# refresh-bio/DSRC

Measured on AMD Instinct MI355X. Metric: raw FASTQ MB/s compressed (bit-identical .dsrc) at -d3 -q2, higher is better.
Workload: dtype u8/u16/u32 integer

## Files before the change

dsrc_amd/csrc/dsrc_gpu.hip:

```cpp
#include <hip/hip_runtime.h>

#include <algorithm>
#include <atomic>
#include <cstdarg>
#include <cstdio>
#include <cstdlib>
#include <cstring>
#include <chrono>
#include <condition_variable>
#include <deque>
#include <functional>
#include <dlfcn.h>
#include <mutex>
#ifndef DSRC_REPLAY_WHATIF
#define DSRC_REPLAY_WHATIF 0
#endif
#include <string>
#include <thread>
#include <vector>

#include "../../include/dsrc_gpu.h"
#include "dsrc_types.h"
#include "k_common.h"
#ifndef RCS_WIDE
// ... 168 lines not shown
	const char* fill = hook_env("DSRC_GPU_DEBUG_FILL");
	if (h->arena.cap >= need) { h->arena.top = 0; h->arena.failed = false; if (fill) HIPCHK(hipMemsetAsync(h->arena.base, atoi(fill), h->arena.cap, h->stream)); return 0; }
	if (h->arena_fixed && need > h->arena_fixed)
		return fail(h, DSRCGPU_E_NOMEM, "batch needs %zu bytes of HBM scratch, arena is fixed at %llu", need, (unsigned long long)h->arena_fixed);
	if (h->arena.base) { HIPCHK(hipFree(h->arena.base)); h->arena.base = nullptr; h->arena.cap = 0; }
	size_t want = h->arena_fixed ? (size_t)h->arena_fixed : need + need / 64;
	hipError_t e;
	{
		static std::mutex alloc_turn[64];
		std::lock_guard<std::mutex> g(alloc_turn[h->device & 63]);
		const auto t0 = std::chrono::steady_clock::now();
		e = hipMalloc((void**)&h->arena.base, want);
		if (getenv("DSRC_GPU_DEBUG")) fprintf(stderr, "[dsrc_gpu] %p arena of %.1f GB: hipMalloc took %.0f ms\n", (void*)h, want / 1e9, std::chrono::duration<double, std::milli>(std::chrono::steady_clock::now() - t0).count());
	}
	if (e != hipSuccess) return fail(h, DSRCGPU_E_NOMEM, "hipMalloc(%zu) for the batch arena failed: %s", want, hipGetErrorString(e));
	h->arena.cap = want; h->arena.top = 0; h->arena.failed = false;
	if (fill) HIPCHK(hipMemsetAsync(h->arena.base, atoi(fill), h->arena.cap, h->stream));
	return 0;
}

u32 bitlen(u64 x) { for (u32 i = 0; i < 32; ++i) if (x < (1ull << i)) return i; return 64; }
u32 log2u(u32 x) { u32 r = 0; while (x > 1) { x >>= 1; ++r; } return r; }
u32 h_huff_ws_words(u32 n) { const u32 m = n < 2 ? 2 : n; return 10 * m; }
u32 h_huff_tree_cap(u32 n) { const u32 m = n < 2 ? 2 : n; return (16 + (2 * m + m * 10) / 8 + 8 + 3) & ~3u; }
size_t al(size_t x, size_t a) { return (x + a - 1) / a * a; }

size_t estimate_arena(const dsrcgpu_handle* h, u32 n, const u64* sizes)
{
	const bool rc = h->set.dna_order > 0 || h->set.quality_order > 0;
	size_t tot = 0, mx = 0;
	for (u32 i = 0; i < n; ++i) { tot += (size_t)sizes[i] + 4096; mx = std::max(mx, (size_t)sizes[i]); }
	const size_t sort_slice = std::min(tot * 14, slice_budget(tot) + mx * 16);
	const size_t copy = (h->set.tag_preserve_flags || h->ds.color_space || !h->rec_pending.empty()) ? tot + (1u << 20) : 0;
	return tot * (h->rc_caps_worst ? 18 : 15) / 2 + (rc ? sort_slice : 0) + (size_t)n * (1u << 20) + (16u << 20) + copy;
}
size_t estimate_decode_arena(const dsrcgpu_handle* h, u32 n, const u64* sizes, bool own_text);

struct BatchIO
{
	const u8* d_in; const u64* offs; const u64* sizes; u32 n;
	u8* d_out; u64 out_cap;
	u8* host_out; u64 host_cap;
	u64* out_offs; u64* out_sizes; u64* raw; u64* comp;
	const std::vector<u32>* layout = nullptr;
	bool in_is_callers = false;
};

template <typename T> T* AP(dsrcgpu_handle* h, size_t off) { return (T*)(h->arena.base + off); }

int run_batch(dsrcgpu_handle* h, BatchIO io)
{
	const u32 B = io.n;
	if (B == 0) return DSRCGPU_OK;
	static const bool trace = getenv("DSRC_GPU_DEBUG") && atoi(getenv("DSRC_GPU_DEBUG")) >= 2;
	const auto t_call = std::chrono::steady_clock::now();
	std::string tl;
	auto mark = [&](const char* what) { if (trace) { char b[64]; snprintf(b, sizeof b, " %s %.1f", what, std::chrono::duration<double, std::milli>(std::chrono::steady_clock::now() - t_call).count()); tl += b; } };
	hipStream_t s = h->stream;
	Arena& A = h->arena;
	h->stage_used = 0; h->stage_kind.clear();
	auto stage_mark = [&](u32 kind)
	{
		if (h->stage_used == h->stage_ev.size()) { hipEvent_t e = nullptr; if (hipEventCreate(&e) != hipSuccess) return; h->stage_ev.push_back(e); }
		(void)hipEventRecord(h->stage_ev[h->stage_used++], s); h->stage_kind.push_back(kind);
	};
	const u32 dna_order = h->set.dna_order, qo = h->set.quality_order;
	const bool lossy = h->set.lossy != 0, crc = h->set.calculate_crc32 != 0;
// ... 8 lines not shown
	if (prm.color_space && (prm.record_layout || prm.tag_flags))
		return fail(h, DSRCGPU_E_ARG, "colour space cannot be combined with the field filter or the record layout on the GPU path");
	if (prm.record_layout && (layout.size() != B || prm.tag_flags || crc))
		return fail(h, DSRCGPU_E_ARG, "record layout: one chunkSize per chunk of the batch, no field filter, no CRC (src/DsrcArchive.cpp:33-47)");

	std::vector<BlkDesc> desc(B);
	std::vector<BlkState> st(B);
	memset(desc.data(), 0, sizeof(BlkDesc) * B);
	size_t in_total = 0;
	for (u32 b = 0; b < B; ++b)
	{
		if (io.sizes[b] == 0 || io.sizes[b] >= (1ull << 31)) return fail(h, DSRCGPU_E_ARG, "chunk %u: size %llu out of range", b, (unsigned long long)io.sizes[b]);
		desc[b].in_off = io.offs[b]; desc[b].in_size = (u32)io.sizes[b];
		if (prm.record_layout) desc[b].chunk_size_value = layout[b];
		desc[b].n_tiles = (u32)((io.sizes[b] + DSRC_TILE_BYTES - 1) / DSRC_TILE_BYTES);
		prm.max_tiles = std::max(prm.max_tiles, desc[b].n_tiles);
		in_total += io.sizes[b];
	}
	const u8* d_in = io.d_in;
	HIPCHK(hipEventRecord(h->ev[0], s));
	if (io.in_is_callers && (prm.tag_flags || prm.color_space || prm.record_layout))
	{
		u64 lo = ~0ull, hi = 0;
		for (u32 b = 0; b < B; ++b) { lo = std::min<u64>(lo, io.offs[b]); hi = std::max<u64>(hi, io.offs[b] + io.sizes[b]); }
		const size_t o_copy = A.alloc(hi - lo + 64);
		if (A.failed) return fail(h, DSRCGPU_E_NOMEM, "arena exhausted (copy of the input)");
		HIPCHK(hipMemcpyAsync(AP<u8>(h, o_copy), io.d_in + lo, hi - lo, hipMemcpyDeviceToDevice, s));
		d_in = AP<u8>(h, o_copy) - lo;
	}
	TraceRange tr; tr.stage("dsrc batch: line index");

	const size_t o_desc = A.alloc(sizeof(BlkDesc) * B), o_state = A.alloc(sizeof(BlkState) * B);
	const size_t o_tiles = A.alloc((size_t)B * prm.max_tiles * 4);
	if (A.failed) return fail(h, DSRCGPU_E_NOMEM, "arena exhausted (phase 1)");
	BlkDesc* d_desc = AP<BlkDesc>(h, o_desc); BlkState* d_state = AP<BlkState>(h, o_state); u32* d_tiles = AP<u32>(h, o_tiles);
	HIPCHK(hipMemcpyAsync(d_desc, desc.data(), sizeof(BlkDesc) * B, hipMemcpyHostToDevice, s));
	HIPCHK(hipMemsetAsync(d_state, 0, sizeof(BlkState) * B, s));
	hipLaunchKernelGGL(k_init_state, dim3((B + 63) / 64), dim3(64), 0, s, d_state, B); KCHK();
	hipLaunchKernelGGL(k_count_lines, dim3(prm.max_tiles, B), dim3(WG), 0, s, d_in, d_desc, d_state, d_tiles, prm); KCHK();
	hipLaunchKernelGGL(k_scan_tiles, dim3(B), dim3(WG), 0, s, d_desc, d_tiles, prm); KCHK();
	HIPCHK(hipMemcpyAsync(st.data(), d_state, sizeof(BlkState) * B, hipMemcpyDeviceToHost, s));
	HIPCHK(hipStreamSynchronize(s));
	mark("S1"); tr.stage("dsrc batch: records, statistics");

	u64 lines = 0, recs = 0; u32 max_rec_cap = 1;
	for (u32 b = 0; b < B; ++b)
	{
		const u32 n_lines = st[b].n_term + 1;
		desc[b].line_base = (u32)lines; lines += n_lines + 2;
		desc[b].rec_cap = (n_lines + 3) / 4;
		desc[b].rec_base = (u32)recs; recs += desc[b].rec_cap + 1;
		max_rec_cap = std::max(max_rec_cap, desc[b].rec_cap);
		if (lines >= (1ull << 32) || recs >= (1ull << 32)) return fail(h, DSRCGPU_E_ARG, "batch too large for 32-bit record indices; submit fewer chunks per batch");
	}
	const size_t o_lines = A.alloc(lines * 4);
	RecPools rp;
	rp.title_off = AP<u32>(h, A.alloc(recs * 4)); rp.seq_off = AP<u32>(h, A.alloc(recs * 4)); rp.qual_off = AP<u32>(h, A.alloc(recs * 4));
	rp.title_len = AP<u16>(h, A.alloc(recs * 2)); rp.len = AP<u16>(h, A.alloc(recs * 2));
	rp.kept = AP<u16>(h, A.alloc(recs * 2)); rp.trunc = AP<u16>(h, A.alloc(recs * 2));
	rp.q_off = AP<u32>(h, A.alloc(recs * 4)); rp.d_off = AP<u32>(h, A.alloc(recs * 4));
	const bool streams_early = prm.tag_flags != 0;
	u8* d_q = nullptr; u8* d_qp = nullptr; u8* d_d = nullptr;
	if (streams_early)
	{
		u64 qbytes = 0;
		for (u32 b = 0; b < B; ++b) { desc[b].q_base = qbytes; desc[b].d_base = qbytes; qbytes += al(desc[b].in_size / 2 + 64, 64); }
		const size_t o_q = A.alloc(qbytes), o_qp = A.alloc(qbytes), o_d = A.alloc(qbytes);
		d_q = AP<u8>(h, o_q); d_qp = AP<u8>(h, o_qp); d_d = AP<u8>(h, o_d);
	}
	if (A.failed) return fail(h, DSRCGPU_E_NOMEM, "arena exhausted (phase 2): need > %zu bytes", A.top);
	u32* d_lines = AP<u32>(h, o_lines);
	HIPCHK(hipMemcpyAsync(d_desc, desc.data(), sizeof(BlkDesc) * B, hipMemcpyHostToDevice, s));
	hipLaunchKernelGGL(k_index_lines, dim3(prm.max_tiles, B), dim3(WG), 0, s, d_in, d_desc, d_tiles, d_lines, prm); KCHK();
	hipLaunchKernelGGL(k_records, dim3((max_rec_cap + WG - 1) / WG, B), dim3(WG), 0, s, d_in, d_desc, d_state, d_lines, rp); KCHK();
	if (prm.tag_flags) { hipLaunchKernelGGL(k_tag_filter, dim3((max_rec_cap + WG - 1) / WG, B), dim3(WG), 0, s, const_cast<u8*>(d_in), d_desc, d_state, rp, prm); KCHK(); }
	const u32 rec_gx = std::max(1u, std::min(64u, (max_rec_cap + 4 * WAVES - 1) / (4 * WAVES)));
	if (prm.color_space)
	{
		hipLaunchKernelGGL(k_rec_count, dim3((B + 63) / 64), dim3(64), 0, s, d_desc, d_state, B); KCHK();
		if (crc) { hipLaunchKernelGGL(k_crc, dim3(B, 3), dim3(WG), 0, s, d_in, d_desc, d_state, rp, h->d_crc_tab, prm); KCHK(); }
		hipLaunchKernelGGL(k_cs_decode, dim3(rec_gx, B), dim3(WG), 0, s, const_cast<u8*>(d_in), d_desc, d_state, rp); KCHK();
	}
	const u32 stats_parts = (u32)hook_int("DSRC_GPU_HOOK_STATS_PARTS", B >= 192 ? 1 : std::min<long>(16, std::max<long>(2, 512 / B)));
	hipLaunchKernelGGL(k_prep_stats, dim3(stats_parts, B), dim3(WG), 0, s, d_in, d_desc, d_state, rp, prm); KCHK();
	if (prm.color_space) { hipLaunchKernelGGL(k_cs_reduce, dim3((max_rec_cap + WG - 1) / WG, B), dim3(WG), 0, s, d_in, d_desc, d_state, rp, prm); KCHK(); }
	hipLaunchKernelGGL(k_rec_offsets, dim3(B), dim3(WG), 0, s, d_desc, d_state, rp); KCHK();
	const u32 prep_gx = std::max(1u, std::min(64u, (max_rec_cap + 4 * WAVES - 1) / (4 * WAVES)));
	if (streams_early) { hipLaunchKernelGGL(k_prep_write, dim3(prep_gx, B), dim3(WG), 0, s, d_in, d_desc, d_state, rp, d_q, d_qp, d_d, prm); KCHK(); }
	if (crc && !prm.color_space) { hipLaunchKernelGGL(k_crc, dim3(B, 3), dim3(WG), 0, s, d_in, d_desc, d_state, rp, h->d_crc_tab, prm); KCHK(); }
	if (prm.tag_flags || prm.record_layout) { hipLaunchKernelGGL(k_tag_poke, dim3((max_rec_cap + WG - 1) / WG, B), dim3(WG), 0, s, const_cast<u8*>(d_in), d_desc, d_state, rp, prm); KCHK(); }
	hipLaunchKernelGGL(k_tag_template, dim3((B + 63) / 64), dim3(64), 0, s, d_in, d_desc, d_state, rp, B); KCHK();
	HIPCHK(hipMemcpyAsync(st.data(), d_state, sizeof(BlkState) * B, hipMemcpyDeviceToHost, s));
	HIPCHK(hipStreamSynchronize(s));
	mark("S2"); tr.stage("dsrc batch: schemes, streams, tag statistics");

	for (u32 b = 0; b < B; ++b)
		if (st[b].err) return fail(h, DSRCGPU_E_INPUT, "chunk %u cannot be coded (error bits 0x%x, %u records)", b, st[b].err, st[b].n_recs);

	if (!streams_early)
	{
		u64 qb = 0, db = 0; bool any_var = false;
		for (u32 b = 0; b < B; ++b)
		{
			desc[b].q_base = qb; qb += al((size_t)st[b].q_total + 64, 64);
			desc[b].d_base = db; db += al((size_t)st[b].d_total + 64, 64);
			any_var = any_var || st[b].min_len != st[b].max_len;
		}
		const size_t o_q = A.alloc(qb + 64), o_d = A.alloc(db + 64), o_qp = any_var ? A.alloc(qb + 64) : 0;
		if (A.failed) return fail(h, DSRCGPU_E_NOMEM, "arena exhausted (symbol streams): need > %zu bytes", A.top);
		d_q = AP<u8>(h, o_q); d_d = AP<u8>(h, o_d); d_qp = any_var ? AP<u8>(h, o_qp) : d_q;
	}

	std::vector<TagPlan> tplan(B);
	std::vector<QuaPlan> qplan(B), dplan(B);
	memset(tplan.data(), 0, sizeof(TagPlan) * B); memset(qplan.data(), 0, sizeof(QuaPlan) * B); memset(dplan.data(), 0, sizeof(QuaPlan) * B);
	std::vector<CtxJob> jobs;
	std::vector<CtxJob> qjobs, djobs;

	static const u32 QN[8] = {16, 32, 64, 128, 16, 32, 64, 128};
	static const u32 ORD1[4] = {3, 2, 1, 1}, ORD2[4] = {4, 3, 2, 1};

// ... 50 lines not shown
			else if ((float)S.raw_len / (float)S.th_len > 1.10f) D.q_scheme = 1;
			else D.q_scheme = 0;
		}
		else if (lossy) D.q_scheme = 0;
		else
		{
			u32 scheme = 255;
			for (u32 i = 0; i < 8; ++i) if ((16u << i) >= S.q_count) { scheme = i; break; }
			if (scheme != 255 && qo == 2)
			{
				const double ratio = (double)S.raw_len / (double)S.rle_len;
				if (S.max_len == S.min_len && ratio > 1.175) scheme += 4;
			}
			if (scheme > 7 || (scheme > 3 && S.q_count > 128)) return fail(h, DSRCGPU_E_INPUT, "chunk %u: %u quality symbols is undefined in the reference's order model", b, S.q_count);
			D.q_scheme = scheme;
		}
	}

	for (u32 b = 0; b < B; ++b)
	{
		const BlkState& S = st[b];
		tplan[b].val = A.alloc((size_t)std::max(1u, S.n_num0) * S.n_recs * 4) / 4;
		tplan[b].rl = A.alloc((size_t)std::max(1u, S.n_num0) * 2 * S.n_recs * 2) / 2;
	}
	const size_t o_tplan = A.alloc(sizeof(TagPlan) * B), o_tres = A.alloc(sizeof(TagFieldRes) * B * DSRC_MAX_FIELDS);
	const size_t o_qplan = A.alloc(sizeof(QuaPlan) * B), o_dplan = A.alloc(sizeof(QuaPlan) * B);
	if (A.failed) return fail(h, DSRCGPU_E_NOMEM, "arena exhausted (phase 3a)");
	TagPlan* d_tplan = AP<TagPlan>(h, o_tplan); TagFieldRes* d_tres = AP<TagFieldRes>(h, o_tres);
	QuaPlan* d_qplan = AP<QuaPlan>(h, o_qplan); QuaPlan* d_dplan = AP<QuaPlan>(h, o_dplan);
	u32* wpool = AP<u32>(h, 0); u64* lpool = AP<u64>(h, 0); u16* spool = AP<u16>(h, 0);

	HIPCHK(hipMemcpyAsync(d_desc, desc.data(), sizeof(BlkDesc) * B, hipMemcpyHostToDevice, s));
	HIPCHK(hipMemcpyAsync(d_tplan, tplan.data(), sizeof(TagPlan) * B, hipMemcpyHostToDevice, s));
	if (!streams_early) { hipLaunchKernelGGL(k_prep_write, dim3(prep_gx, B), dim3(WG), 0, s, d_in, d_desc, d_state, rp, d_q, d_qp, d_d, prm); KCHK(); }
	hipLaunchKernelGGL(k_tag_scan, dim3(stats_parts, B), dim3(WG), 0, s, d_in, d_desc, d_state, rp, wpool, d_tplan); KCHK();
	hipLaunchKernelGGL(k_tag_numeric, dim3(B), dim3(WG), 0, s, d_desc, d_state, wpool, spool, d_tplan); KCHK();
	hipLaunchKernelGGL(k_tag_finalize, dim3(B), dim3(64), 0, s, d_state); KCHK();

	size_t zero_lo = al(A.top, 256); A.top = zero_lo;
	for (u32 b = 0; b < B; ++b)
	{
		const BlkState& S = st[b]; BlkDesc& D = desc[b];
		if (qo == 0)
		{
			QuaPlan& P = qplan[b];
			P.scheme = D.q_scheme; P.blk = b;
			size_t cap_bytes;
			if (D.q_scheme <= 1)
			{
				const u32 hw = S.max_len * S.q_count;
				P.hist_words = hw; P.code_off = hw; P.len_off = 2 * hw;
				P.tree_slot = 4 + h_huff_tree_cap(S.q_count); P.tree_off = 3 * hw;
				P.n_trees = S.max_len;
				const u32 tree_words = (u32)(((size_t)S.max_len * P.tree_slot + 3) / 4);
				P.ws_slot = h_huff_ws_words(S.q_count); P.ws_off = P.tree_off + tree_words;
				P.aux_off = P.ws_off + S.max_len * P.ws_slot;
				const size_t words = (size_t)P.aux_off + S.n_recs + 4;
				P.scr = A.alloc(words * 4) / 4;
				cap_bytes = 64 + (size_t)S.max_len * P.tree_slot + ((size_t)S.q_total * (bitlen(S.q_count) + 1) + 7) / 8 + (size_t)S.n_recs * 3;
			}
			else
			{
				const u32 qn = S.q_count, hw = qn * qn + qn * 256;
				P.hist_words = hw; P.code_off = hw; P.len_off = 2 * hw; P.lf_off = 3 * hw;
				P.tree_slot = 4 + h_huff_tree_cap(256); P.tree_off = P.lf_off + 256; P.n_trees = 2 * qn;
				const u32 tree_words = (u32)(((size_t)2 * qn * P.tree_slot + 3) / 4);
				P.ws_slot = h_huff_ws_words(256); P.ws_off = P.tree_off + tree_words;
// ... 297 lines not shown
		if (use_bk) HIPCHK(hipMemsetAsync(d_bk, 0, bk_zero_words * 4, s));
		const u32 max_parts = 2048u;
		launch_fallback = [&, sort_atomic, max_parts](const BkGroup& g) -> int
		{
			const u32 cnt = g.hi - g.lo;
			const u32* fb = d_bk + g.fb;
			if (sort_atomic) hipLaunchKernelGGL((k_sort<0, true>), dim3(std::min(cnt, 16u)), dim3(SORT_WG), 0, s, d_jobs, lpool, d_d, d_q, d_qp, d_state, fb);
			else hipLaunchKernelGGL((k_sort<0, false>), dim3(std::min(cnt, 16u)), dim3(SORT_WG), 0, s, d_jobs, lpool, d_d, d_q, d_qp, d_state, fb);
			u32 mxn = 1; for (u32 i = g.lo; i < g.hi; ++i) mxn = std::max(mxn, jobs[i].n);
			const u32 parts = std::max(1u, std::min(max_parts, mxn / 1024u));
			const dim3 rgrid(parts * std::min(cnt, 4u));
#define BK_REPLAY(NN) { hipLaunchKernelGGL(k_replay_seams<NN>, rgrid, dim3(REPLAY_WG), 0, s, d_jobs, const_cast<u64*>(lpool), parts, cnt, fb); \
					hipLaunchKernelGGL((k_replay<NN, 0>), rgrid, dim3(REPLAY_WG), 0, s, d_jobs, lpool, AP<RcPack>(h, 0), parts, cnt, fb); }
			switch (jobs[g.lo].n_alpha)
			{
			case 4: BK_REPLAY(4) break; case 8: BK_REPLAY(8) break; case 16: BK_REPLAY(16) break;
			case 32: BK_REPLAY(32) break; case 64: BK_REPLAY(64) break; default: BK_REPLAY(128) break;
			}
#undef BK_REPLAY
			KCHK();
			return 0;
		};
		for (size_t sl = 0; sl + 1 < slice_lo.size(); ++sl)
		{
			const u32 s_lo = slice_lo[sl], s_hi = slice_lo[sl + 1];
			stage_mark(0);
			if (use_bk)
			{
				u32 slice_bins = 0;
				for (u32 i = s_lo; i < s_hi; ++i) if (jobs[i].bk_on) slice_bins = std::max(slice_bins, (jobs[i].n + BK_BIN - 1) >> BK_TB);
				hipLaunchKernelGGL(k_part, dim3(std::max(1u, slice_bins), s_hi - s_lo), dim3(PART_WG), 0, s, d_jobs + s_lo, lpool, d_d, d_q, d_qp, d_state, d_bk, d_bcnt);
				KCHK();
				stage_mark(0); stage_mark(1);
				if (slice_bins) { hipLaunchKernelGGL(k_binoff, dim3(slice_bins, s_hi - s_lo), dim3(256), 0, s, d_jobs + s_lo, d_bcnt, d_bk); KCHK(); }
				for (const BkGroup& g : bk_groups[sl])
				{
					u32 hb = 0; bool any = false;
					for (u32 i = g.lo; i < g.hi; ++i) if (jobs[i].bk_on) { any = true; hb = std::max(hb, jobs[i].bk_hb); }
					if (!any) continue;
					u32 lbm = 0; for (u32 i = g.lo; i < g.hi; ++i) if (jobs[i].bk_on) lbm = std::max(lbm, jobs[i].bk_lb);
#define BK_LAUNCH(NN, MB, RB) hipLaunchKernelGGL((k_model<NN, MB, RB>), dim3(((1u << hb) + MD_WAVES_FOR(RB) - 1) / MD_WAVES_FOR(RB), g.hi - g.lo), dim3(64 * MD_WAVES_FOR(RB)), 0, s, d_jobs + g.lo, lpool, AP<RcPack>(h, 0), d_bk, d_bcnt, (RcPack*)(d_bk + ((bk_zero_words + 1) & ~(size_t)1)))
#define BK_FINISH(NN) { if ((1u << lbm) * 4 * MdRow<NN>::STRIDE <= 4096) BK_LAUNCH(NN, 0, 4096); \
						else if ((1u << lbm) * 4 * MdRow<NN>::STRIDE <= MD_ROW_BYTES) BK_LAUNCH(NN, 0, MD_ROW_BYTES); \
						else if (lbm <= 10) BK_LAUNCH(NN, 10, MD_ROW_BYTES); \
						else BK_LAUNCH(NN, BK_MAX_LB, MD_ROW_BYTES); }
					switch (jobs[g.lo].n_alpha)
					{
					case 4: BK_FINISH(4) break; case 8: BK_FINISH(8) break; case 16: BK_FINISH(16) break;
					case 32: BK_FINISH(32) break; case 64: BK_FINISH(64) break; default: BK_FINISH(128) break;
					}
#undef BK_LAUNCH
#undef BK_FINISH
					KCHK();
				}
				if (bk_binned && slice_bins) { hipLaunchKernelGGL(k_place, dim3(slice_bins, s_hi - s_lo), dim3(PLACE_WG), 0, s, d_jobs + s_lo, lpool, AP<RcPack>(h, 0), d_bk); KCHK(); }
				for (const BkGroup& g : bk_groups[sl])
				{
					bool known = false;
					for (u32 i = g.lo; i < g.hi; ++i) known = known || !jobs[i].bk_on;
					if (known) { const int rc = launch_fallback(g); if (rc) return rc; }
				}
				stage_mark(1);
				continue;
			}
#ifdef DSRC_SORT_PROBE
			{
				static int shots = 0;
// ... 1493 lines not shown
```

dsrc_amd/csrc/k_bucket.h:

```cpp
#pragma once
#include <type_traits>
#include "k_rc.h"

#define BK_MAX_HB 10
#define BK_MAX_LB 11
#define BK_LIMIT 524288
#define BK_BIG 16384
#ifndef BK_TB
#define BK_TB 13
#endif
#define BK_BIN (1u << BK_TB)
static_assert(BK_TB == RC6_TB, "a time bin is the unit of k_rc's record layout (rc6_chunk_off)");
#ifndef BK_MAX_BINS
#define BK_MAX_BINS 512
#endif
#define BK_MAX_BINS_WIDE 65536
#define BK_HASH_MUL 0x9E3779B1u


__device__ __forceinline__ u64 bk_rekey(const CtxJob& j, u64 el)
{
	const u32 key = ((u32)(el >> ELEM_CTX_SHIFT) * j.bk_mul) & j.bk_kmask;
	return (el & ((1ull << ELEM_CTX_SHIFT) - 1ull)) | ((u64)key << ELEM_CTX_SHIFT);
}
// ... 131 lines not shown
			}
		}
	}
	if (bad) atomicOr(&st[j.blk].err, (u32)DSRC_ERR_REF_UB);
	const u32 shift = 7 + lb;
#pragma unroll
	for (u32 k = 0; k < PART_ITEMS; ++k)
	{
		const u32 i = wbase + k * 64 + lane;
		const u32 d = ks[k] >> shift;
		const u32 sh = (d & 1u) * 16u;
		u32 old = 0;
		if (i < n) old = atomicAdd(&((u32*)s_cnt[wv])[d >> 1], 1u << sh);
		rk[k] = (old >> sh) & 0xFFFFu;
#ifdef DSRC_EMU_BUILD
		(void)__ballot(true);
#endif
	}
	__syncthreads();
	for (u32 d0 = 0, carry = 0; d0 < bins; d0 += PART_WG)
	{
		const u32 dd = d0 + threadIdx.x;
		u32 c[PART_WAVES], tot = 0;
#pragma unroll
		for (u32 w = 0; w < PART_WAVES; ++w) { c[w] = dd < bins ? s_cnt[w][dd] : 0u; tot += c[w]; }
		const u32 inc = wave_incl_scan_dpp(tot);
		if (lane == 63) s_ws[wv] = inc;
		__syncthreads();
		u32 run = carry + inc - tot;
		const u32 nws = (bins - d0 + 63) / 64 < PART_WAVES ? (bins - d0 + 63) / 64 : PART_WAVES;
		for (u32 i = 0; i < nws; ++i) { const u32 x = s_ws[i]; run += i < wv ? x : 0u; carry += x; }
		if (dd < bins)
		{
			bcnt[(u64)j.bk_cnt + (u64)blockIdx.x * bins + dd] = (u16)tot;
#pragma unroll
			for (u32 w = 0; w < PART_WAVES; ++w) { s_cnt[w][dd] = (u16)run; run += c[w]; }
		}
		if (d0 + PART_WG < bins) __syncthreads();
	}
	__syncthreads();
	const u32 lbmask = (1u << lb) - 1u;
	u32* dst = (u32*)(pool + j.elems) + tile;
	const u32 tile_n = n - tile < tile_elems ? n - tile : tile_elems;
	constexpr u32 PIECE = BK_BIN / PART_PASSES;
#pragma unroll
	for (u32 k = 0; k < PART_ITEMS; ++k) rk[k] += (u32)s_cnt[wv][ks[k] >> shift];
#pragma unroll
	for (u32 p = 0; p < PART_PASSES; ++p)
	{
#pragma unroll
		for (u32 k = 0; k < PART_ITEMS; ++k)
		{
			const u32 i = wbase + k * 64 + lane;
			const u32 at = rk[k] - p * PIECE;
			if (i < n && at < PIECE)
				s_tile[at] = (((ks[k] >> 7) & lbmask) << BK_EL_KEY_SHIFT) | ((ks[k] & 0x7Fu) << BK_EL_SYM_SHIFT) | (i & (BK_BIN - 1u));
		}
		__syncthreads();
		if (tile_n == tile_elems)
		{
#pragma unroll
			for (u32 k = 0; k < PIECE / 2 / PART_WG; ++k) ((u64*)(dst + p * PIECE))[k * PART_WG + threadIdx.x] = ((const u64*)s_tile)[k * PART_WG + threadIdx.x];
		}
		else for (u32 q = threadIdx.x; q < PIECE && p * PIECE + q < tile_n; q += PART_WG) dst[p * PIECE + q] = s_tile[q];
		if (p + 1 < PART_PASSES) __syncthreads();
	}
}
// ... 61 lines not shown
					if (l == G::L4 - 1) { const u32 p = row[2 * G::W64 + c]; sum = (p & 0xFFFFu) + (p >> 16); }
					else { const u64 o = r64[((1u << (2 * (l + 1))) - 1u) / 3u + c]; sum = ((u32)o & 0xFFFFu) + ((u32)o >> 16) + ((u32)(o >> 32) & 0xFFFFu) + (u32)(o >> 48); }
					v |= (u64)sum << (16 * q);
				}
			}
			r64[base + w] = v;
		}
	}
}

template <int N> __device__ __forceinline__ u64 md_code(u32* row, u32 sym)
{
	typedef MdRow<N> G;
	unsigned long long* r64 = (unsigned long long*)row;
	u32 cum = 0, tot = 0, f = 0;
#pragma unroll
	for (int l = 0; l < G::L4; ++l)
	{
		const u32 q = (sym >> (G::B - 2 * l - 2)) & 3u;
		const u32 wi = ((1u << (2 * l)) - 1u) / 3u + (l ? sym >> (G::B - 2 * l) : 0u);
		const u64 old = atomicAdd(&r64[wi], 2ull << (16 * q));
		const u64 below = old & ((1ull << (16 * q)) - 1ull);
		cum += ((u32)below & 0xFFFFu) + ((u32)below >> 16) + ((u32)(below >> 32) & 0xFFFFu);
		if (l == 0) tot = ((u32)old & 0xFFFFu) + ((u32)old >> 16) + ((u32)(old >> 32) & 0xFFFFu) + (u32)(old >> 48);
		f = (u32)(old >> (16 * q)) & 0xFFFFu;
	}
	if (G::R2)
	{
		const u32 old = atomicAdd(&row[2 * G::W64 + (sym >> 1)], (sym & 1u) ? (2u << 16) : 2u);
		cum += (sym & 1u) ? (old & 0xFFFFu) : 0u;
		f = (sym & 1u) ? (old >> 16) : (old & 0xFFFFu);
	}
	return (u64)f | ((u64)cum << 16) | ((u64)tot << 32);
}

__global__ void __launch_bounds__(256) k_binoff(const CtxJob* jobs, u16* bcnt, const u32* bk)
{
	const CtxJob j = jobs[blockIdx.y];
	const u32 bin = blockIdx.x;
	if (!j.bk_on || bk[j.jid] || (bin << BK_TB) >= j.n) return;
	const u32 bins = 1u << j.bk_hb;
	u16* row = bcnt + j.bk_cnt + (u64)bin * bins;
	u32 c[4], mine = 0;
#pragma unroll
	for (u32 k = 0; k < 4; ++k)
	{
		const u32 b = 4 * threadIdx.x + k;
		c[k] = b < bins ? (u32)row[b] : 0u;
		mine += c[k];
	}
	u32 tot;
	u32 run = block_excl_scan(mine, &tot);
#pragma unroll
	for (u32 k = 0; k < 4; ++k)
	{
		const u32 b = 4 * threadIdx.x + k;
		if (b < bins) row[b] = (u16)run;
		run += c[k];
	}
}

template <bool SMALL> struct MdMapT { typedef u8 T; static constexpr u32 NONE = 0xFFu, CLAIM = 0x80u; };
template <> struct MdMapT<false> { typedef u16 T; static constexpr u32 NONE = 0xFFFFu, CLAIM = 0x8000u; };

#ifndef MD_AHEAD
#define MD_AHEAD 3
#endif
#ifndef MD_ROTATE_ALL
#define MD_ROTATE_ALL 0
#endif
template <int N, int MAPBITS, int ROW_BYTES>
__global__ void __launch_bounds__(64 * MD_WAVES_FOR(ROW_BYTES)) k_model(const CtxJob* jobs, const u64* pool, RcPack* rec_pool, u32* bk, const u16* bcnt, RcPack* nowhere)
{
	constexpr u32 STRIDE = MdRow<N>::STRIDE;
	constexpr u32 ROWS = ROW_BYTES / (4 * STRIDE);
	constexpr u32 MD_WAVES = MD_WAVES_FOR(ROW_BYTES);
	typedef MdMapT<(ROWS <= 127)> Map;
	typedef typename Map::T map_t;
	__shared__ map_t s_map[MD_WAVES][1 << MAPBITS];
	__shared__ unsigned long long s_rows[MD_WAVES][ROW_BYTES / 8];
	__shared__ u16 s_off[MD_WAVES][BK_MAX_BINS];
	__shared__ u16 s_num[MD_WAVES][BK_MAX_BINS];
	__shared__ u8 s_head[MD_WAVES][64];
	constexpr u32 limit = (1u << 16) - 2u * N;
	const CtxJob j = jobs[blockIdx.y];
	const u32 w = wave_id(), lane = lane_id();
#ifndef MD_XCD_MAP
#define MD_XCD_MAP 1
#endif
	u32 bx = blockIdx.x;
	if (MD_XCD_MAP && gridDim.x % 8u == 0) bx = (((bx & 7u) + blockIdx.y) & 7u) * (gridDim.x >> 3) + (bx >> 3);
	const u32 bucket = bx * MD_WAVES + w;
// ... 256 lines not shown
```

dsrc_amd/csrc/k_parse.h:

```cpp
#pragma once
#include "k_common.h"

typedef u64 __attribute__((aligned(1))) u64_text;

__device__ __forceinline__ u32 byte_eq8(u64 w, u64 c_rep)
{
	const u64 x = w ^ c_rep;
	const u64 y = (((x & 0x7F7F7F7F7F7F7F7Full) + 0x7F7F7F7F7F7F7F7Full) | x) | 0x7F7F7F7F7F7F7F7Full;
	return (u32)((((~y) >> 7) * 0x0102040810204080ull) >> 56);
}

struct LineBits { u64 term, crlf; };

__device__ __forceinline__ LineBits classify64(const u8* p, u64 base, u64 size)
{
	LineBits r; r.term = 0; r.crlf = 0;
	if (base >= size) return r;
	u64 lf = 0, cr = 0;
	if (base + DSRC_LANE_BYTES <= size)
	{
#pragma unroll
		for (u32 k = 0; k < DSRC_LANE_BYTES / 8; ++k)
		{
			const u64 w = *(const u64_text*)(p + base + 8 * k);
			lf |= (u64)byte_eq8(w, 0x0A0A0A0A0A0A0A0Aull) << (8 * k);
			cr |= (u64)byte_eq8(w, 0x0D0D0D0D0D0D0D0Dull) << (8 * k);
		}
	}
	else
	{
		for (u32 k = 0; base + k < size; ++k)
		{
			const u8 c = p[base + k];
			if (c == '\n') lf |= 1ull << k;
			if (c == '\r') cr |= 1ull << k;
		}
	}
	const u64 n_valid = size - base;
	const u64 valid = n_valid >= 64 ? ~0ull : ((1ull << n_valid) - 1ull);
	const bool lf_next = base + DSRC_LANE_BYTES < size && p[base + DSRC_LANE_BYTES] == '\n';
	const bool cr_prev = base > 0 && p[base - 1] == '\r';
	const u64 lf_after = (lf >> 1) | (lf_next ? 1ull << 63 : 0ull);
	const u64 cr_before = (cr << 1) | (cr_prev ? 1ull : 0ull);
	r.term = (lf | (cr & ~lf_after)) & valid;
	r.crlf = (lf & cr_before) & valid;
	return r;
}

__global__ void __launch_bounds__(WG) k_count_lines(const u8* in, const BlkDesc* desc, BlkState* st, u32* tile_cnt, DsrcParams prm)
{
	__shared__ u32 s_tot[2];
	const u32 b = blockIdx.y, tile = blockIdx.x;
	const BlkDesc d = desc[b];
	if (tile >= d.n_tiles) return;
	if (threadIdx.x < 2) s_tot[threadIdx.x] = 0;
	__syncthreads();
	const LineBits lb = classify64(in + d.in_off, (u64)tile * DSRC_TILE_BYTES + (u64)threadIdx.x * DSRC_LANE_BYTES, d.in_size);
	const u32 cnt = wave_sum((u32)__popcll(lb.term)), crlf = wave_sum((u32)__popcll(lb.crlf));
	if (lane_id() == 0) { if (cnt) atomicAdd(&s_tot[0], cnt); if (crlf) atomicAdd(&s_tot[1], crlf); }
	__syncthreads();
	if (threadIdx.x == 0)
	{
		tile_cnt[(u64)b * prm.max_tiles + tile] = s_tot[0];
		atomicAdd(&st[b].n_term, s_tot[0]);
		if (s_tot[1]) atomicAdd(&st[b].n_crlf, s_tot[1]);
	}
}

__global__ void __launch_bounds__(WG) k_scan_tiles(const BlkDesc* desc, u32* tile_cnt, DsrcParams prm)
{
	const u32 b = blockIdx.x;
	const u32 n = desc[b].n_tiles;
	u32* t = tile_cnt + (u64)b * prm.max_tiles;
	u32 carry = 0;
	for (u32 base = 0; base < n; base += blockDim.x)
	{
		const u32 i = base + threadIdx.x;
		const u32 v = i < n ? t[i] : 0;
		u32 tot;
		const u32 ex = block_excl_scan(v, &tot);
		if (i < n) t[i] = carry + ex;
		carry += tot;
	}
}

__global__ void __launch_bounds__(WG) k_index_lines(const u8* in, const BlkDesc* desc, const u32* tile_base, u32* line_start, DsrcParams prm)
{
	const u32 b = blockIdx.y, tile = blockIdx.x;
	const BlkDesc d = desc[b];
	if (tile >= d.n_tiles) return;
	const u64 base = (u64)tile * DSRC_TILE_BYTES + (u64)threadIdx.x * DSRC_LANE_BYTES;
	const LineBits lb = classify64(in + d.in_off, base, d.in_size);
	u64 mask = lb.term;
	u32 total;
	u32 rank = block_excl_scan((u32)__popcll(mask), &total) + tile_base[(u64)b * prm.max_tiles + tile];
	u32* ls = line_start + d.line_base;
	if (tile == 0 && threadIdx.x == 0) ls[0] = 0;
	while (mask)
	{
		const u32 k = (u32)__ffsll((long long)mask) - 1;
		mask &= mask - 1;
		ls[++rank] = (u32)(base + k + 1) | ((u32)((lb.crlf >> k) & 1ull) << 31);
	}
}

struct RecPools
{
	u32* title_off; u32* seq_off; u32* qual_off;
	u16* title_len; u16* len;
	u16* kept; u16* trunc;
	u32* q_off; u32* d_off;
};

#define LS_POS(x) ((x) & 0x7FFFFFFFu)
__device__ __forceinline__ void line_extent(const u32* ls, u32 n_term, u32 size, u32 i, u32* start, u32* len)
{
	if (i > n_term) { *start = size; *len = 0; return; }
	const u32 s = LS_POS(ls[i]);
	*start = s;
	if (i == n_term) { *len = size - s; return; }
	const u32 nx = ls[i + 1];
	const u32 e = LS_POS(nx) - 1 - (nx >> 31);
	*len = e - s;
}

// ... 87 lines not shown
}
__device__ __forceinline__ void dna_index_table(u8* lut) { for (u32 i = threadIdx.x; i < 256; i += blockDim.x) lut[i] = (u8)dna_index(i); }
__device__ __forceinline__ u32 transform_base_s(u32 s, u32 qual, u32 qoff, u32 lossy, u32* sidx, bool* keep)
{
	*sidx = s;
	u32 q;
	if (!lossy)
	{
		q = (qual - qoff) & 255u;
		if (s > 3 && q < 7) { q = (q + 128u + ((s - 2u) << 3) - 16u) & 255u; *keep = false; }
		else *keep = true;
	}
	else
	{
		q = lossy_bin((qual - qoff) & 255u);
		if (s >= 4) { q = 0; *keep = false; }
		else { if (q == 0) q = 1; *keep = true; }
	}
	return q;
}

__device__ __forceinline__ u32 block_rec_count(const BlkState& S, const BlkDesc& d)
{
	u32 n_cand = (S.n_term + 1 + 3) / 4;
	if (n_cand > d.rec_cap) n_cand = d.rec_cap;
	return S.first_bad < n_cand ? S.first_bad : n_cand;
}

__global__ void __launch_bounds__(64) k_rec_count(const BlkDesc* desc, BlkState* st, u32 n_blocks)
{
	const u32 b = blockIdx.x * blockDim.x + threadIdx.x;
	if (b < n_blocks) st[b].n_recs = block_rec_count(st[b], desc[b]);
}

__device__ __forceinline__ u32 cs_state(u32 c) { return c == 'C' ? 1u : c == 'G' ? 2u : c == 'T' ? 3u : 0u; }

__global__ void __launch_bounds__(WG) k_cs_decode(u8* in, const BlkDesc* desc, BlkState* st, RecPools rp)
{
	const u32 b = blockIdx.y;
	const BlkDesc d = desc[b];
	u8* p = in + d.in_off;
	const u32 n_recs = st[b].n_recs;
	const u32 lane = lane_id();
	const u32 waves_total = gridDim.x * (blockDim.x >> 6);
	for (u32 r = blockIdx.x * (blockDim.x >> 6) + wave_id(); r < n_recs; r += waves_total)
	{
		const u64 g = (u64)d.rec_base + r;
		const u32 len = rp.len[g], so = rp.seq_off[g];
		if (len == 0) continue;
		if (lane == 0 && p[so] != p[rp.seq_off[d.rec_base]]) atomicOr(&st[b].cs_varbegin, 1u);
		u32 state = cs_state(p[so]);
		bool bad = false;
		for (u32 j0 = 0; j0 < len; j0 += 64)
		{
			const u32 j = j0 + lane;
			const bool in_r = j < len && j >= 1;
			const u32 c = in_r ? (u32)p[so + j] - '.' : 0u;
			if (c > 5) bad = true;
			const u32 col = (in_r && c >= 2 && c <= 5) ? c - 2 : 0u;
			const u64 m0 = __ballot((col & 1u) != 0), m1 = __ballot((col & 2u) != 0);
			const u64 le = lanemask_lt() | (1ull << lane);
			const u32 mine = state ^ ((u32)__popcll(m0 & le) & 1u) ^ (((u32)__popcll(m1 & le) & 1u) << 1);
			if (in_r) p[so + j] = c < 2 ? (u8)'N' : (u8)"ACGT"[mine];
			state ^= ((u32)__popcll(m0) & 1u) ^ (((u32)__popcll(m1) & 1u) << 1);
		}
		if (bad) atomicOr(&st[b].err, (u32)DSRC_ERR_BAD_BASE);
// ... 269 lines not shown
```

Before: 65760.

## Cache line-terminator maps, fold bin-offset scan into partition, shrink prep workgroups

```diff
diff --git a/dsrc_amd/csrc/dsrc_gpu.hip b/dsrc_amd/csrc/dsrc_gpu.hip
--- a/dsrc_amd/csrc/dsrc_gpu.hip
+++ b/dsrc_amd/csrc/dsrc_gpu.hip
@@ -224,7 +224,8 @@
 	for (u32 i = 0; i < n; ++i) { tot += (size_t)sizes[i] + 4096; mx = std::max(mx, (size_t)sizes[i]); }
 	const size_t sort_slice = std::min(tot * 14, slice_budget(tot) + mx * 16);
 	const size_t copy = (h->set.tag_preserve_flags || h->ds.color_space || !h->rec_pending.empty()) ? tot + (1u << 20) : 0;
-	return tot * (h->rc_caps_worst ? 18 : 15) / 2 + (rc ? sort_slice : 0) + (size_t)n * (1u << 20) + (16u << 20) + copy;
+	const size_t term_maps = (size_t)n * ((mx + DSRC_TILE_BYTES - 1) / DSRC_TILE_BYTES) * (DSRC_TILE_BYTES / 8);
+	return tot * (h->rc_caps_worst ? 18 : 15) / 2 + (rc ? sort_slice : 0) + (size_t)n * (1u << 20) + (16u << 20) + copy + term_maps;
 }
 size_t estimate_decode_arena(const dsrcgpu_handle* h, u32 n, const u64* sizes, bool own_text);
 
@@ -299,12 +300,13 @@
 
 	const size_t o_desc = A.alloc(sizeof(BlkDesc) * B), o_state = A.alloc(sizeof(BlkState) * B);
 	const size_t o_tiles = A.alloc((size_t)B * prm.max_tiles * 4);
+	const size_t o_term = A.alloc((size_t)B * prm.max_tiles * WG * 8);
 	if (A.failed) return fail(h, DSRCGPU_E_NOMEM, "arena exhausted (phase 1)");
-	BlkDesc* d_desc = AP<BlkDesc>(h, o_desc); BlkState* d_state = AP<BlkState>(h, o_state); u32* d_tiles = AP<u32>(h, o_tiles);
+	BlkDesc* d_desc = AP<BlkDesc>(h, o_desc); BlkState* d_state = AP<BlkState>(h, o_state); u32* d_tiles = AP<u32>(h, o_tiles); u64* d_term = AP<u64>(h, o_term);
 	HIPCHK(hipMemcpyAsync(d_desc, desc.data(), sizeof(BlkDesc) * B, hipMemcpyHostToDevice, s));
 	HIPCHK(hipMemsetAsync(d_state, 0, sizeof(BlkState) * B, s));
 	hipLaunchKernelGGL(k_init_state, dim3((B + 63) / 64), dim3(64), 0, s, d_state, B); KCHK();
-	hipLaunchKernelGGL(k_count_lines, dim3(prm.max_tiles, B), dim3(WG), 0, s, d_in, d_desc, d_state, d_tiles, prm); KCHK();
+	hipLaunchKernelGGL(k_count_lines, dim3(prm.max_tiles, B), dim3(WG), 0, s, d_in, d_desc, d_state, d_tiles, d_term, prm); KCHK();
 	hipLaunchKernelGGL(k_scan_tiles, dim3(B), dim3(WG), 0, s, d_desc, d_tiles, prm); KCHK();
 	HIPCHK(hipMemcpyAsync(st.data(), d_state, sizeof(BlkState) * B, hipMemcpyDeviceToHost, s));
 	HIPCHK(hipStreamSynchronize(s));
@@ -338,22 +340,23 @@
 	if (A.failed) return fail(h, DSRCGPU_E_NOMEM, "arena exhausted (phase 2): need > %zu bytes", A.top);
 	u32* d_lines = AP<u32>(h, o_lines);
 	HIPCHK(hipMemcpyAsync(d_desc, desc.data(), sizeof(BlkDesc) * B, hipMemcpyHostToDevice, s));
-	hipLaunchKernelGGL(k_index_lines, dim3(prm.max_tiles, B), dim3(WG), 0, s, d_in, d_desc, d_tiles, d_lines, prm); KCHK();
+	hipLaunchKernelGGL(k_index_lines, dim3(prm.max_tiles, B), dim3(WG), 0, s, d_in, d_desc, d_state, d_tiles, d_term, d_lines, prm); KCHK();
 	hipLaunchKernelGGL(k_records, dim3((max_rec_cap + WG - 1) / WG, B), dim3(WG), 0, s, d_in, d_desc, d_state, d_lines, rp); KCHK();
 	if (prm.tag_flags) { hipLaunchKernelGGL(k_tag_filter, dim3((max_rec_cap + WG - 1) / WG, B), dim3(WG), 0, s, const_cast<u8*>(d_in), d_desc, d_state, rp, prm); KCHK(); }
-	const u32 rec_gx = std::max(1u, std::min(64u, (max_rec_cap + 4 * WAVES - 1) / (4 * WAVES)));
+	constexpr u32 PREP_WAVES = PREP_WG / 64;
+	const u32 rec_gx = std::max(1u, std::min(64u * (WG / PREP_WG), (max_rec_cap + 4 * PREP_WAVES - 1) / (4 * PREP_WAVES)));
 	if (prm.color_space)
 	{
 		hipLaunchKernelGGL(k_rec_count, dim3((B + 63) / 64), dim3(64), 0, s, d_desc, d_state, B); KCHK();
 		if (crc) { hipLaunchKernelGGL(k_crc, dim3(B, 3), dim3(WG), 0, s, d_in, d_desc, d_state, rp, h->d_crc_tab, prm); KCHK(); }
-		hipLaunchKernelGGL(k_cs_decode, dim3(rec_gx, B), dim3(WG), 0, s, const_cast<u8*>(d_in), d_desc, d_state, rp); KCHK();
+		hipLaunchKernelGGL(k_cs_decode, dim3(rec_gx, B), dim3(PREP_WG), 0, s, const_cast<u8*>(d_in), d_desc, d_state, rp); KCHK();
 	}
 	const u32 stats_parts = (u32)hook_int("DSRC_GPU_HOOK_STATS_PARTS", B >= 192 ? 1 : std::min<long>(16, std::max<long>(2, 512 / B)));
 	hipLaunchKernelGGL(k_prep_stats, dim3(stats_parts, B), dim3(WG), 0, s, d_in, d_desc, d_state, rp, prm); KCHK();
 	if (prm.color_space) { hipLaunchKernelGGL(k_cs_reduce, dim3((max_rec_cap + WG - 1) / WG, B), dim3(WG), 0, s, d_in, d_desc, d_state, rp, prm); KCHK(); }
 	hipLaunchKernelGGL(k_rec_offsets, dim3(B), dim3(WG), 0, s, d_desc, d_state, rp); KCHK();
-	const u32 prep_gx = std::max(1u, std::min(64u, (max_rec_cap + 4 * WAVES - 1) / (4 * WAVES)));
-	if (streams_early) { hipLaunchKernelGGL(k_prep_write, dim3(prep_gx, B), dim3(WG), 0, s, d_in, d_desc, d_state, rp, d_q, d_qp, d_d, prm); KCHK(); }
+	const u32 prep_gx = rec_gx;
+	if (streams_early) { hipLaunchKernelGGL(k_prep_write, dim3(prep_gx, B), dim3(PREP_WG), 0, s, d_in, d_desc, d_state, rp, d_q, d_qp, d_d, prm); KCHK(); }
 	if (crc && !prm.color_space) { hipLaunchKernelGGL(k_crc, dim3(B, 3), dim3(WG), 0, s, d_in, d_desc, d_state, rp, h->d_crc_tab, prm); KCHK(); }
 	if (prm.tag_flags || prm.record_layout) { hipLaunchKernelGGL(k_tag_poke, dim3((max_rec_cap + WG - 1) / WG, B), dim3(WG), 0, s, const_cast<u8*>(d_in), d_desc, d_state, rp, prm); KCHK(); }
 	hipLaunchKernelGGL(k_tag_template, dim3((B + 63) / 64), dim3(64), 0, s, d_in, d_desc, d_state, rp, B); KCHK();
@@ -470,7 +473,7 @@
 
 	HIPCHK(hipMemcpyAsync(d_desc, desc.data(), sizeof(BlkDesc) * B, hipMemcpyHostToDevice, s));
 	HIPCHK(hipMemcpyAsync(d_tplan, tplan.data(), sizeof(TagPlan) * B, hipMemcpyHostToDevice, s));
-	if (!streams_early) { hipLaunchKernelGGL(k_prep_write, dim3(prep_gx, B), dim3(WG), 0, s, d_in, d_desc, d_state, rp, d_q, d_qp, d_d, prm); KCHK(); }
+	if (!streams_early) { hipLaunchKernelGGL(k_prep_write, dim3(prep_gx, B), dim3(PREP_WG), 0, s, d_in, d_desc, d_state, rp, d_q, d_qp, d_d, prm); KCHK(); }
 	hipLaunchKernelGGL(k_tag_scan, dim3(stats_parts, B), dim3(WG), 0, s, d_in, d_desc, d_state, rp, wpool, d_tplan); KCHK();
 	hipLaunchKernelGGL(k_tag_numeric, dim3(B), dim3(WG), 0, s, d_desc, d_state, wpool, spool, d_tplan); KCHK();
 	hipLaunchKernelGGL(k_tag_finalize, dim3(B), dim3(64), 0, s, d_state); KCHK();
@@ -834,7 +837,6 @@
 				hipLaunchKernelGGL(k_part, dim3(std::max(1u, slice_bins), s_hi - s_lo), dim3(PART_WG), 0, s, d_jobs + s_lo, lpool, d_d, d_q, d_qp, d_state, d_bk, d_bcnt);
 				KCHK();
 				stage_mark(0); stage_mark(1);
-				if (slice_bins) { hipLaunchKernelGGL(k_binoff, dim3(slice_bins, s_hi - s_lo), dim3(256), 0, s, d_jobs + s_lo, d_bcnt, d_bk); KCHK(); }
 				for (const BkGroup& g : bk_groups[sl])
 				{
 					u32 hb = 0; bool any = false;
diff --git a/dsrc_amd/csrc/k_bucket.h b/dsrc_amd/csrc/k_bucket.h
--- a/dsrc_amd/csrc/k_bucket.h
+++ b/dsrc_amd/csrc/k_bucket.h
@@ -187,7 +187,7 @@
 		for (u32 i = 0; i < nws; ++i) { const u32 x = s_ws[i]; run += i < wv ? x : 0u; carry += x; }
 		if (dd < bins)
 		{
-			bcnt[(u64)j.bk_cnt + (u64)blockIdx.x * bins + dd] = (u16)tot;
+			bcnt[(u64)j.bk_cnt + (u64)blockIdx.x * bins + dd] = (u16)run;
 #pragma unroll
 			for (u32 w = 0; w < PART_WAVES; ++w) { s_cnt[w][dd] = (u16)run; run += c[w]; }
 		}
@@ -315,32 +315,6 @@
 		f = (sym & 1u) ? (old >> 16) : (old & 0xFFFFu);
 	}
 	return (u64)f | ((u64)cum << 16) | ((u64)tot << 32);
-}
-
-__global__ void __launch_bounds__(256) k_binoff(const CtxJob* jobs, u16* bcnt, const u32* bk)
-{
-	const CtxJob j = jobs[blockIdx.y];
-	const u32 bin = blockIdx.x;
-	if (!j.bk_on || bk[j.jid] || (bin << BK_TB) >= j.n) return;
-	const u32 bins = 1u << j.bk_hb;
-	u16* row = bcnt + j.bk_cnt + (u64)bin * bins;
-	u32 c[4], mine = 0;
-#pragma unroll
-	for (u32 k = 0; k < 4; ++k)
-	{
-		const u32 b = 4 * threadIdx.x + k;
-		c[k] = b < bins ? (u32)row[b] : 0u;
-		mine += c[k];
-	}
-	u32 tot;
-	u32 run = block_excl_scan(mine, &tot);
-#pragma unroll
-	for (u32 k = 0; k < 4; ++k)
-	{
-		const u32 b = 4 * threadIdx.x + k;
-		if (b < bins) row[b] = (u16)run;
-		run += c[k];
-	}
 }
 
 template <bool SMALL> struct MdMapT { typedef u8 T; static constexpr u32 NONE = 0xFFu, CLAIM = 0x80u; };
diff --git a/dsrc_amd/csrc/k_parse.h b/dsrc_amd/csrc/k_parse.h
--- a/dsrc_amd/csrc/k_parse.h
+++ b/dsrc_amd/csrc/k_parse.h
@@ -47,7 +47,9 @@
 	return r;
 }
 
-__global__ void __launch_bounds__(WG) k_count_lines(const u8* in, const BlkDesc* desc, BlkState* st, u32* tile_cnt, DsrcParams prm)
+__device__ __forceinline__ u64 term_map_at(u32 b, u32 tile, u32 max_tiles) { return ((u64)b * max_tiles + tile) * WG + threadIdx.x; }
+
+__global__ void __launch_bounds__(WG) k_count_lines(const u8* in, const BlkDesc* desc, BlkState* st, u32* tile_cnt, u64* term_map, DsrcParams prm)
 {
 	__shared__ u32 s_tot[2];
 	const u32 b = blockIdx.y, tile = blockIdx.x;
@@ -56,6 +58,7 @@
 	if (threadIdx.x < 2) s_tot[threadIdx.x] = 0;
 	__syncthreads();
 	const LineBits lb = classify64(in + d.in_off, (u64)tile * DSRC_TILE_BYTES + (u64)threadIdx.x * DSRC_LANE_BYTES, d.in_size);
+	term_map[term_map_at(b, tile, prm.max_tiles)] = lb.term;
 	const u32 cnt = wave_sum((u32)__popcll(lb.term)), crlf = wave_sum((u32)__popcll(lb.crlf));
 	if (lane_id() == 0) { if (cnt) atomicAdd(&s_tot[0], cnt); if (crlf) atomicAdd(&s_tot[1], crlf); }
 	__syncthreads();
@@ -84,13 +87,15 @@
 	}
 }
 
-__global__ void __launch_bounds__(WG) k_index_lines(const u8* in, const BlkDesc* desc, const u32* tile_base, u32* line_start, DsrcParams prm)
+__global__ void __launch_bounds__(WG) k_index_lines(const u8* in, const BlkDesc* desc, const BlkState* st, const u32* tile_base, const u64* term_map, u32* line_start, DsrcParams prm)
 {
 	const u32 b = blockIdx.y, tile = blockIdx.x;
 	const BlkDesc d = desc[b];
 	if (tile >= d.n_tiles) return;
 	const u64 base = (u64)tile * DSRC_TILE_BYTES + (u64)threadIdx.x * DSRC_LANE_BYTES;
-	const LineBits lb = classify64(in + d.in_off, base, d.in_size);
+	LineBits lb;
+	if (st[b].n_crlf == 0) { lb.term = term_map[term_map_at(b, tile, prm.max_tiles)]; lb.crlf = 0; }
+	else lb = classify64(in + d.in_off, base, d.in_size);
 	u64 mask = lb.term;
 	u32 total;
 	u32 rank = block_excl_scan((u32)__popcll(mask), &total) + tile_base[(u64)b * prm.max_tiles + tile];
@@ -244,6 +249,12 @@
 	const u32 b = blockIdx.x * blockDim.x + threadIdx.x;
 	if (b < n_blocks) st[b].n_recs = block_rec_count(st[b], desc[b]);
 }
+
+#ifndef DSRC_PREP_WG
+#define DSRC_PREP_WG (DSRC_WG < 256 ? DSRC_WG : 256)
+#endif
+#define PREP_WG DSRC_PREP_WG
+static_assert(PREP_WG % 64 == 0 && PREP_WG <= WG && WG % PREP_WG == 0, "whole waves, within the kernels' launch bounds");
 
 __device__ __forceinline__ u32 cs_state(u32 c) { return c == 'C' ? 1u : c == 'G' ? 2u : c == 'T' ? 3u : 0u; }
 
```

After: 68040, median of 6. +3.5%, better.
